# ray-project/kuberay

Measured on NVIDIA H100. Metric: reconciles/sec over 10k RayCluster x 100 pods (batched reconcilePods + status roll-up), higher is better.
Workload: dtype u32

## Files before the change

kuberay_b200/csrc/kr_bucket2.cuh:

```cuda
#pragma once

#include "kr_decide.cuh"

namespace kr {

__device__ __forceinline__ uint32_t inc_epoch_of(const ScratchDev &sc) { return __ldcg(&sc.inc[KR_INC_EPOCH]) + 1u; }

#ifndef KR_D2WARPS
#define KR_D2WARPS 8
#endif
static constexpr int kD2Warps = KR_D2WARPS;
#define KR_ROW_UNHEALTHY (1u << 13)
#define KR_ROW_FRESH (1u << 14)
#define KR_LG_OWNED (1u << 31)

__device__ __forceinline__ uint4 *large_slot(const ScratchDev &sc, uint32_t c, uint32_t rank) {
  if (!sc.lg) return nullptr;
  const uint4 l = __ldcg(&sc.lg[c]);
  const uint32_t j = rank - sc.bucket_stride;
  return j < l.y ? sc.region + l.x + j : nullptr;
}
__device__ __forceinline__ uint4 *rec_slot(const ScratchDev &sc, uint32_t c, uint32_t rank) {
  return rank < sc.bucket_stride ? sc.bucket + (size_t)c * sc.bucket_stride + rank : large_slot(sc, c, rank);
}
// ... 181 lines not shown
    if ((int64_t)count < (int64_t)H) {
#pragma unroll
      for (int k = 0; k < K; k++) if ((mine >> k) & 1u) act[k] = KR_ACT_DELETE_MH_INCOMPLETE;
      gr.flags |= KR_GR_ABORTED; err_arg = (int32_t)count;
      return KR_ERR_MH_INCOMPLETE;
    }
    if (name == KR_ID_EMPTY_STRING) r_empty = n_rep;
    n_rep++;
  }
  for (uint32_t r = lane; r < n_rep; r += 32) s_rep[r] = 0;
  __syncwarp();
#pragma unroll
  for (int k = 0; k < K; k++) {
    if ((((labelled | noname) >> k) & 1u) && (pw[k] & KR_ROW_UNHEALTHY)) {
      const uint32_t r = ((noname >> k) & 1u) ? r_empty : rep[k];
      if (r != KR_MH_NONE) atomicOr(&s_rep[r], KR_MHF_DELETED);
    }
  }
  __syncwarp();
  int32_t n_unh = 0;
#pragma unroll
  for (int k = 0; k < K; k++) {
    const bool hit = ((labelled >> k) & 1u) && (s_rep[rep[k]] & KR_MHF_DELETED);
    if (hit) act[k] = KR_ACT_DELETE_MH_UNHEALTHY;
    n_unh += __popc(__ballot_sync(0xFFFFFFFFu, hit));
  }
  gr.n_unhealthy = n_unh;
  if (wtd_cnt > 0) {
#pragma unroll
    for (int k = 0; k < K; k++) {
      if ((((labelled | noname) >> k) & 1u) && (pw[k] & KR_ROW_WTD_OWN)) {
        const uint32_t r = ((noname >> k) & 1u) ? r_empty : rep[k];
        if (r != KR_MH_NONE) atomicOr(&s_rep[r], KR_MHF_WTD);
      }
    }
    __syncwarp();
    int32_t n_del = 0;
#pragma unroll
    for (int k = 0; k < K; k++) {
      const bool hit = ((labelled >> k) & 1u) && (s_rep[rep[k]] & KR_MHF_WTD);
      if (hit && act[k] == KR_ACT_KEEP) act[k] = KR_ACT_DELETE_MH_WTD;
      n_del += __popc(__ballot_sync(0xFFFFFFFFu, hit));
    }
    gr.flags |= KR_GR_WTD_EXECUTED;
    if (n_del > 0) { gr.flags |= KR_GR_ABORTED; err_arg = n_del; return KR_ERR_MH_WTD; }
  }
  int32_t running = 0;
  for (uint32_t r = lane; r < n_rep; r += 32) running += (s_rep[r] & KR_MHF_DELETED) ? 0 : 1;
  running = __reduce_add_sync(0xFFFFFFFFu, running);
#pragma unroll
  for (int k = 0; k < K; k++) if (((heads >> k) & 1u) && !(s_rep[rep[k]] & KR_MHF_DELETED)) mh_head |= 1u << k;
  gr.n_running = running;
  if (expected % H != 0) { gr.flags |= KR_GR_ABORTED; err_arg = expected; return KR_ERR_MH_NOT_MULTIPLE; }
  const int32_t to_create = expected / H - running;
  gr.diff = to_create;
  if (to_create > 0) gr.n_create = (uint32_t)to_create;
  else if (to_create < 0) {
    if (delete_allowed) {
      const int32_t remove = -to_create;
      int32_t seen = 0;
      for (uint32_t b = 0; b < n_rep && seen < remove; b += 32) {
        const uint32_t r = b + lane;
        const bool ok = r < n_rep && !(s_rep[r] & KR_MHF_DELETED);
        const uint32_t bal = __ballot_sync(0xFFFFFFFFu, ok);
        if (ok && seen + (int32_t)__popc(bal & lt) < remove) s_rep[r] |= KR_MHF_SCALE;
        seen += __popc(bal);
      }
      __syncwarp();
#pragma unroll
      for (int k = 0; k < K; k++) if (((labelled >> k) & 1u) && (s_rep[rep[k]] & KR_MHF_SCALE)) act[k] = KR_ACT_DELETE_MH_SCALE_DOWN;
    } else gr.flags |= KR_GR_RANDOM_DELETE_OFF;
  }
  return KR_ERR_NONE;
}

template <int K, bool kInc = false, bool kMH = false>
__global__ void __launch_bounds__(kD2Warps * 32, (K <= 4 && !kMH ? 32 : 16) / kD2Warps) k_decide2(Decide2Args a) {
  const int phase = kInc ? 2 : a.phase;
  KR_TL(phase ? 12 : 3);
  __shared__ int32_t s_acc[kD2Warps][3][KR_SMEM_GROUPS];
  __shared__ int32_t s_mode[kD2Warps][kMH ? 4 : 3][KR_SMEM_GROUPS];
  __shared__ uint32_t s_list[kD2Warps][32 * K];
  __shared__ uint32_t s_bits[kD2Warps][32];
  const SnapDev &s = a.s;
  const uint32_t warp = threadIdx.x >> 5, lane = threadIdx.x & 31;
  const uint32_t lt = lanemask_lt();
  const uint32_t S = a.sc.bucket_stride;
  uint32_t c = blockIdx.x * kD2Warps + warp;
  bool mine = phase == 0 && c < a.n.n_clusters;
  RecordCI ci{mine ? __ldg(&a.sc.cl_in[32 * (size_t)c + lane]) : 0u};
  pdl_wait(); pdl_trigger();
  if (phase == 1) {
    mine = c < a.r.totals[4];
    if (mine) { c = a.sc.deferred_list[c]; ci.word = __ldg(&a.sc.cl_in[32 * (size_t)c + lane]); }
  } else if (kInc) {
    mine = c < __ldcg(&a.sc.inc[KR_INC_DIRTY]) && !__ldcg(&a.sc.inc[KR_INC_VOID]) && !__ldcg(&a.sc.inc[KR_INC_STRUCTURAL]);
    if (mine) {
      c = a.sc.dirty_list[c];
      ci.word = __ldcg(&a.sc.cl_in[32 * (size_t)c + lane]);
    }
  }
  if (KR_ATTEMPT_VOID(a.r.totals)) mine = false;
  if (ci.group_cnt() > KR_SMEM_GROUPS) mine = false;
  if (kInc && !mine) return;
  uint4 *bucket = a.sc.bucket + (size_t)(mine ? c : 0) * S;
  uint4 dyn = make_uint4(0, 0, 0, 0);
  uint4 recs[K] = {};
  if (mine) {
    dyn = __ldcg(&a.sc.cl_dyn[c]);
#pragma unroll
    for (int k = 0; k < K; k++) if ((uint32_t)(k * 32) + lane < S) recs[k] = __ldcg(&bucket[k * 32 + lane]);
  }
  uint32_t P = dyn.x;
  if (P > S) { mine = false; P = 0; }
  if (kInc) {
    const uint32_t epoch = inc_epoch_of(a.sc);
    const bool lost = dyn.y == epoch;
    uint32_t kept = 0, head_min = 0xFFFFFFFFu;
#pragma unroll
    for (int k = 0; k < K; k++) {
      const uint32_t j = k * 32 + lane;
      bool keep = mine && j < P;
      const bool fresh = keep && (recs[k].y & KR_ROW_FRESH);
      if (keep && lost && !fresh) keep = __ldcg(&a.sc.stamp[recs[k].x]) != epoch;
      const uint32_t bal = __ballot_sync(0xFFFFFFFFu, keep);
      if (keep) {
        uint4 rec = recs[k];
        rec.y &= ~KR_ROW_FRESH;
        const uint32_t to = kept + __popc(bal & lt);
        if (fresh || to != j) { bucket[to] = rec; if (to != j) a.sc.pos[rec.x] = to; }
        if (pp_node_type(rec.y & 0xFFFFu) == KR_NT_HEAD) head_min = min(head_min, rec.x);
      }
      kept += __popc(bal);
    }
    head_min = __reduce_min_sync(0xFFFFFFFFu, head_min);
    __syncwarp();
    unsigned long long raw = 0;
    if (mine) {
      if (lane == 0 && head_min != 0xFFFFFFFFu) raw = ~(((unsigned long long)head_min << 32) | (uint32_t)(aux_lookup(a.sc, head_min) + 1));
      raw = __shfl_sync(0xFFFFFFFFu, raw, 0);
      P = kept;
      dyn = make_uint4(kept, 0u, (uint32_t)raw, (uint32_t)(raw >> 32));
      if (lane == 0) a.sc.cl_dyn[c] = dyn;
#pragma unroll
      for (int k = 0; k < K; k++) if ((uint32_t)(k * 32) + lane < kept) recs[k] = __ldcg(&bucket[k * 32 + lane]);
    }
  }
  const uint32_t cf = ci.flags(), G = ci.group_cnt(), g0 = ci.group_off();
  const uint8_t suspend_status = ci.suspend_status(), ext_err = ci.ext_err_kind(), old_prov = ci.cond_status(KR_COND_PROVISIONED);
  const bool gate = a.f.gate_status_conditions != 0;
  uint32_t old_create = 0;
  if (kInc && mine) {
    for (uint32_t gi = lane; gi < G; gi += 32) old_create += a.r.groups[g0 + gi].n_create;
    old_create = __reduce_add_sync(0xFFFFFFFFu, old_create);
  }
  uint32_t head_pod = 0xFFFFFFFFu;
  int32_t head_aux = -1;
  {
    const unsigned long long raw = ((unsigned long long)dyn.w << 32) | dyn.z;
    if (mine && raw != 0) { const unsigned long long key = ~raw; head_pod = (uint32_t)(key >> 32); head_aux = (int32_t)(uint32_t)key - 1; }
  }
  uint8_t h_ver = KR_VER_EMPTY, h_ast = KR_ANNOT_EMPTY;
  if (head_aux >= 0 && (cf & KR_CF_UPGRADE_RECREATE)) { h_ver = s.h_version_state[head_aux]; h_ast = s.h_annot_state[head_aux]; }
  uint32_t pidx[K], pw[K], ridx[K], act[K];
  uint32_t head_pos = 0xFFFFFFFFu, head_name = 0, head_flags = 0;
#pragma unroll
  for (int k = 0; k < K; k++) {
    const uint32_t i = k * 32 + lane;
    const bool valid = i < P;
    pidx[k] = valid ? recs[k].x : 0xFFFFFFFFu; pw[k] = valid ? recs[k].y : (KR_ROW_NO_GROUP << 16); ridx[k] = valid ? recs[k].z : 0u; act[k] = KR_ACT_KEEP;
    const uint32_t hit = __ballot_sync(0xFFFFFFFFu, valid && recs[k].x == head_pod);
    if (hit) {
      const int src = __ffs(hit) - 1;
      head_pos = k * 32 + src;
      head_name = __shfl_sync(0xFFFFFFFFu, recs[k].w, src); head_flags = __shfl_sync(0xFFFFFFFFu, recs[k].y, src) & 0xFFFFu;
    }
  }
  (void)head_pos;
  int32_t *acc_list = s_acc[warp][0], *acc_unh = s_acc[warp][1], *acc_wtd = s_acc[warp][2];
  int32_t *g_mode = s_mode[warp][0], *g_prefix = s_mode[warp][1], *g_ncreate = s_mode[warp][2], *g_mh_running = s_mode[warp][kMH ? 3 : 2];
  uint32_t mh_head = 0;
  if (lane < KR_SMEM_GROUPS) { acc_list[lane] = 0; acc_unh[lane] = 0; acc_wtd[lane] = 0; g_mode[lane] = GM_UNPROCESSED; g_prefix[lane] = 0; g_ncreate[lane] = 0; }
  __syncwarp();

  int32_t ready = 0, available = 0, n_heads = 0, n0_list = 0, n0_unh = 0, n0_wtd = 0;
  bool all_running = P > 0;
  const uint32_t nchunks = (P + 31) / 32;
#pragma unroll
  for (int k = 0; k < K; k++) {
    if ((uint32_t)k >= nchunks) break;
    const bool valid = (uint32_t)(k * 32) + lane < P;
    const uint32_t w = pw[k], fl = w & 0xFFFFu, slot = valid ? (w >> 16) : KR_ROW_NO_GROUP;
    const uint32_t nt = pp_node_type(fl), ph = pp_phase(fl), rd = pp_ready(fl);
    const bool w_run = valid && nt == KR_NT_WORKER && ph == KR_PHASE_RUNNING;
    available += __popc(__ballot_sync(0xFFFFFFFFu, w_run));
    ready += __popc(__ballot_sync(0xFFFFFFFFu, w_run && rd == KR_COND_TRUE));
    const bool not_ok = valid && (ph != KR_PHASE_RUNNING || rd == KR_COND_FALSE || rd == KR_COND_UNKNOWN);
    if (__any_sync(0xFFFFFFFFu, not_ok)) all_running = false;
    n_heads += __popc(__ballot_sync(0xFFFFFFFFu, valid && nt == KR_NT_HEAD));
    if (G == 1) {
      const bool in0 = slot == 0;
      n0_list += __popc(__ballot_sync(0xFFFFFFFFu, in0));
      n0_unh += __popc(__ballot_sync(0xFFFFFFFFu, in0 && (fl & KR_ROW_UNHEALTHY)));
      n0_wtd += __popc(__ballot_sync(0xFFFFFFFFu, in0 && (fl & KR_ROW_WTD_OWN)));
      continue;
    }
    const uint32_t gkey = (slot < G) ? slot : KR_ROW_NO_GROUP;
    const uint32_t peers = __match_any_sync(0xFFFFFFFFu, gkey);
    if (gkey != KR_ROW_NO_GROUP) {
      const uint32_t ub = __ballot_sync(peers, (fl & KR_ROW_UNHEALTHY) != 0);
      const uint32_t wb = __ballot_sync(peers, (fl & KR_ROW_WTD_OWN) != 0);
      if ((peers & lt) == 0) {
        acc_list[gkey] += __popc(peers);
        acc_unh[gkey] += __popc(ub & peers);
        acc_wtd[gkey] += __popc(wb & peers);
      }
    }
    __syncwarp();
  }
  if (G == 1) { if (lane == 0) { acc_list[0] = n0_list; acc_unh[0] = n0_unh; acc_wtd[0] = n0_wtd; } __syncwarp(); }

  kr_cluster_result cr;
  {
    uint32_t *z = reinterpret_cast<uint32_t *>(&cr);
#pragma unroll
    for (int k = 0; k < (int)(sizeof(cr) / 4); k++) z[k] = 0;
  }
  cr.head_pod_idx = -1; cr.stop_after_group = -1;
  uint8_t all_action = KR_ACT_KEEP;
  bool head_delete = false, run_groups = false, deferred = false, any_prefix = false;
  uint32_t n_create_cluster = 0;
  if (mine) {
    if (cf & KR_CF_SKIP) {
      cr.path = KR_PATH_SKIPPED;
    } else if (ext_err != KR_EXT_ERR_NONE) {
      cr.path = KR_PATH_SKIPPED;
      cr.err_kind = ext_err == KR_EXT_ERR_STATUS_ONLY_NIL ? KR_ERR_NONE : KR_ERR_EXTERNAL;
    } else if (suspend_status == KR_SUSPEND_SUSPENDING || (!gate && (cf & KR_CF_SUSPEND))) {
      cr.path = KR_PATH_SUSPENDING_DELETE_ALL; all_action = KR_ACT_DELETE_ALL_SUSPEND;
    } else if (gate && (suspend_status == KR_SUSPEND_SUSPENDED || (cf & KR_CF_SUSPEND))) {
      cr.path = KR_PATH_SUSPENDED_NOOP;
    } else {
      bool recreate = false;
      if ((cf & KR_CF_UPGRADE_RECREATE) && n_heads > 0) {
        const int32_t aux = head_aux;
        const uint8_t ver = h_ver, ast = h_ast;
        if (ver == KR_VER_DIFFERENT) cr.head_update_annotations = 1;
        else if (ast == KR_ANNOT_OTHER) recreate = true;
        else if (ast == KR_ANNOT_HASH32 && !a.f.skip_hash) {
          if (phase == 0 && !a.spin_hash) {
            deferred = true;
            if (lane == 0) a.sc.deferred_list[atomicAdd(&a.r.totals[4], 1u)] = c;
          } else {
            const uint8_t *ah = s.h_annot_hash + 32 * (size_t)aux;
            const uint32_t *hw = reinterpret_cast<const uint32_t *>(a.r.hash + 32 * (size_t)c);
            if (phase == 0) {
              if (lane == 0) {
                const volatile uint32_t *w7 = hw + 7;
                uint32_t it = 0;
                while (*w7 == 0u && it < 40000u) { __nanosleep(100); it++; }
                if (*w7 == 0u) atomicOr(&a.r.totals[3], KR_TOTALS_HASH_WAIT);
              }
              __syncwarp();
              __threadfence();
            }
            const uint32_t word = __ldcg(&hw[lane >> 2]);
            recreate = __any_sync(0xFFFFFFFFu, ah[lane] != (uint8_t)(word >> (8 * (lane & 3))));
          }
        }
      }
      if (recreate) {
        cr.path = KR_PATH_RECREATE_DELETE_ALL; all_action = KR_ACT_DELETE_ALL_RECREATE;
      } else {
        cr.path = KR_PATH_NORMAL;
        if (!(cf & KR_CF_HEAD_EXPECT_OK)) { cr.head_action = KR_HEAD_EXPECT_PENDING; run_groups = true; }
        else if (n_heads == 1) {
          if (head_flags & KR_ROW_UNHEALTHY) { cr.head_action = KR_HEAD_DELETE; cr.err_kind = KR_ERR_HEAD_DELETED; head_delete = true; }
          else run_groups = true;
        } else if (n_heads == 0) {
          if (old_prov == KR_COND_TRUE && (cf & KR_CF_SKIP_HEAD_RESTART)) cr.head_action = KR_HEAD_SKIP_RESTART;
          else { cr.head_action = KR_HEAD_CREATE; run_groups = true; }
        } else {
          cr.head_action = KR_HEAD_MULTIPLE; cr.err_kind = KR_ERR_MULTIPLE_HEADS; cr.err_arg = n_heads;
        }
      }
    }
    if (run_groups) {
      const bool autoscaling = (cf & KR_CF_AUTOSCALING) != 0;
      cr.stop_after_group = (int32_t)G;
      for (uint32_t gi = 0; gi < G; gi++) {
        const uint32_t g = g0 + gi;
        const bool rec0 = gi == 0;
        const uint32_t gf = rec0 ? ci.g0_flags() : LDG(s.g_flags[g]);
        const int32_t hosts = rec0 ? ci.g0_hosts() : LDG(s.g_num_hosts[g]), g_rep = rec0 ? ci.g0_rep() : LDG(s.g_replicas[g]);
        const int32_t g_mn = rec0 ? ci.g0_min() : LDG(s.g_min[g]), g_mx = rec0 ? ci.g0_max() : LDG(s.g_max[g]);
        kr_group_result gr;
        gr.expected = 0; gr.n_list = 0; gr.n_unhealthy = 0; gr.n_running = 0; gr.diff = 0; gr.n_create = 0; gr.create_off = 0;
        gr.flags = KR_GR_PROCESSED;
        int32_t mode = GM_SKIP, prefix = 0;
        bool abort_here = false;
        if (!(gf & KR_GF_EXPECT_OK)) {
          gr.flags |= KR_GR_EXPECT_PENDING;
        } else {
          const int32_t expected = desired_replicas(g_rep, g_mn, g_mx, hosts, gf);
          const int32_t n_list = acc_list[gi], n_unh = acc_unh[gi], n_wtd = acc_wtd[gi];
          gr.expected = expected; gr.n_list = n_list;
          if (gf & KR_GF_SUSPEND) { gr.flags |= KR_GR_SUSPENDED; mode = GM_SUSPENDED; }
          else if (kMH && hosts > 1 && a.f.gate_multihost_indexing) {
            gr.flags |= KR_GR_MULTIHOST; mode = GM_MULTIHOST;
            int32_t earg = 0;
            const int ek = decide_multihost2<K>(s, gi, expected, hosts, !autoscaling || a.f.env_random_pod_delete, LDG(s.g_wtd_cnt[g]), pidx, pw, act, mh_head,
                                                s_list[warp], gr, earg, lane);
            if (ek != KR_ERR_NONE) { cr.err_kind = (uint8_t)ek; cr.err_arg = earg; abort_here = true; }
            if (lane == 0) g_mh_running[gi] = gr.n_running;
          }
          else if (n_unh > 0) {
            gr.n_unhealthy = n_unh; gr.flags |= KR_GR_ABORTED; mode = GM_UNHEALTHY;
            cr.err_kind = KR_ERR_UNHEALTHY_WORKERS; cr.err_arg = n_unh; abort_here = true;
          } else {
            gr.flags |= KR_GR_WTD_EXECUTED; mode = GM_NORMAL;
            const int32_t running = n_list - n_wtd;
            const int32_t diff = expected - running;
            gr.n_running = running; gr.diff = diff;
            if (diff > 0) gr.n_create = (uint32_t)diff;
            else if (diff < 0) {
              if (!autoscaling || a.f.env_random_pod_delete) {
                const long long remove = -(long long)diff;
                if (remove > running) {
                  prefix = running; gr.flags |= KR_GR_ABORTED;
                  cr.err_kind = KR_ERR_NEGATIVE_EXPECTED; cr.err_arg = expected; abort_here = true;
                } else prefix = (int32_t)remove;
              } else gr.flags |= KR_GR_RANDOM_DELETE_OFF;
            }
          }
        }
        any_prefix |= prefix > 0;
        n_create_cluster += gr.n_create;
        __syncwarp();
        if (lane == 0) {
          g_mode[gi] = mode; g_prefix[gi] = prefix; g_ncreate[gi] = (int32_t)gr.n_create;
          a.r.groups[g] = gr;
        }
        if (abort_here) { cr.stop_after_group = (int32_t)gi; break; }
      }
    }
    {
      const int32_t reached = ((cf & KR_CF_SKIP) || !run_groups) ? 0 : (cr.stop_after_group == (int32_t)G ? (int32_t)G : cr.stop_after_group + 1);
      for (uint32_t gi = reached + lane; gi < G; gi += 32) {
        kr_group_result z; z.expected = 0; z.n_list = 0; z.n_unhealthy = 0; z.n_running = 0; z.diff = 0; z.n_create = 0; z.create_off = 0; z.flags = 0;
        a.r.groups[g0 + gi] = z;
      }
    }
  }
  __syncwarp();

  uint32_t cand = 0;
  if (mine) {
#pragma unroll
    for (int k = 0; k < K; k++) {
      if ((uint32_t)k >= nchunks) break;
      const bool valid = (uint32_t)(k * 32) + lane < P;
      const uint32_t w = pw[k], fl = w & 0xFFFFu;
      const uint32_t gkey = (valid && run_groups && (w >> 16) < G) ? (w >> 16) : KR_ROW_NO_GROUP;
      const int32_t mode = (gkey != KR_ROW_NO_GROUP) ? g_mode[gkey] : GM_UNPROCESSED;
      uint32_t ac = KR_ACT_KEEP;
      if (all_action != KR_ACT_KEEP) ac = valid ? all_action : (uint32_t)KR_ACT_KEEP;
      else if (head_delete) { if (valid && pidx[k] == head_pod) ac = KR_ACT_DELETE_HEAD; }
      else if (mode == GM_SUSPENDED) ac = KR_ACT_DELETE_GROUP_SUSPEND;
      else if (kMH && mode == GM_MULTIHOST) ac = act[k];
      else if (mode == GM_UNHEALTHY) { if (fl & KR_ROW_UNHEALTHY) ac = KR_ACT_DELETE_UNHEALTHY; }
      else if (mode == GM_NORMAL) {
        if (fl & KR_ROW_WTD_OWN) ac = KR_ACT_DELETE_WTD;
        else cand |= 1u << k;
      }
      act[k] = ac;
    }
    if (any_prefix) {
      for (uint32_t gi = 0; gi < G; gi++) {
        const int32_t pre = g_prefix[gi];
        if (pre <= 0) continue;
        if (pre <= 8) {
          for (int32_t it = 0; it < pre; it++) {
            uint32_t m = 0xFFFFFFFFu;
#pragma unroll
            for (int k = 0; k < K; k++)
              if (((cand >> k) & 1u) && (pw[k] >> 16) == gi && act[k] == KR_ACT_KEEP) m = min(m, pidx[k]);
            const uint32_t wm = __reduce_min_sync(0xFFFFFFFFu, m);
            if (wm == 0xFFFFFFFFu) break;
#pragma unroll
            for (int k = 0; k < K; k++)
              if (((cand >> k) & 1u) && pidx[k] == wm) act[k] = KR_ACT_DELETE_RANDOM;
          }
        } else {
          uint32_t nc = 0;
#pragma unroll
          for (int k = 0; k < K; k++) {
            const bool isc = ((cand >> k) & 1u) && (pw[k] >> 16) == gi;
            const uint32_t bal = __ballot_sync(0xFFFFFFFFu, isc);
            if (isc) s_list[warp][nc + __popc(bal & lt)] = pidx[k];
            nc += __popc(bal);
          }
          __syncwarp();
#pragma unroll
          for (int k = 0; k < K; k++) {
            const bool isc = ((cand >> k) & 1u) && (pw[k] >> 16) == gi;
            if (!__any_sync(0xFFFFFFFFu, isc)) continue;
            uint32_t rank = 0;
            for (uint32_t i = 0; i < nc; i++) rank += s_list[warp][i] < pidx[k] ? 1u : 0u;
            if (isc && (int32_t)rank < pre) act[k] = KR_ACT_DELETE_RANDOM;
          }
          __syncwarp();
        }
      }
    }
  }
  uint32_t n_act = 0;
  uint32_t arank[K];
#pragma unroll
  for (int k = 0; k < K; k++) {
    arank[k] = 0;
    const bool isa = act[k] != KR_ACT_KEEP;
    const uint32_t bal = __ballot_sync(0xFFFFFFFFu, isa);
    if (isa) s_list[warp][n_act + __popc(bal & lt)] = pidx[k];
    n_act += __popc(bal);
  }
  __syncwarp();
  if (n_act > 1) {
#pragma unroll
    for (int k = 0; k < K; k++) {
      const bool isa = act[k] != KR_ACT_KEEP;
      if (!__any_sync(0xFFFFFFFFu, isa)) continue;
      uint32_t rank = 0;
      for (uint32_t i = 0; i < n_act; i++) rank += s_list[warp][i] < pidx[k] ? 1u : 0u;
      arank[k] = rank;
    }
  }

  if (!(cf & KR_CF_SKIP))
    status_rollup(a.s, a.f, ci, cr, P, (uint32_t)n_heads, n_heads > 0 ? (int32_t)head_pod : -1, head_aux, head_name, ready, available, all_running);
  if (mine && lane == 0) a.r.clusters[c] = cr;

  const uint32_t slots = deferred ? P : n_act;
  uint32_t act_off = 0, create_off = 0;
  if (phase == 0) {
    unsigned long long base = 0;
    if (mine && lane == 0) {
      if (slots | n_create_cluster) base = atomicAdd(reinterpret_cast<unsigned long long *>(&a.r.totals[8]), ((unsigned long long)n_create_cluster << 32) | slots);
      if (n_act) atomicAdd(&a.r.totals[2], n_act);
      if (n_create_cluster) atomicAdd(&a.r.totals[6], n_create_cluster);
    }
    base = __shfl_sync(0xFFFFFFFFu, base, 0);
    act_off = (uint32_t)base; create_off = (uint32_t)(base >> 32);
    if (mine && lane == 0) {
      a.r.act_start[c] = act_off; a.r.act_cnt[c] = n_act;
      if (deferred) a.sc.cact[c] = n_create_cluster;
      a.sc.act_res[c] = slots; a.sc.cre_res[c] = n_create_cluster;
    }
  } else if (kInc) {
    unsigned long long base = 0;
    uint32_t need = 0;
    if (mine && lane == 0) {
      const uint32_t old_act = a.r.act_cnt[c];
      need = (n_act > a.sc.act_res[c] ? 1u : 0u) | (n_create_cluster > a.sc.cre_res[c] ? 2u : 0u);
      if (need) base = atomicAdd(reinterpret_cast<unsigned long long *>(&a.r.totals[8]), ((unsigned long long)((need & 2u) ? n_create_cluster : 0u) << 32) | ((need & 1u) ? n_act : 0u));
      if ((need & 1u) && (uint64_t)(uint32_t)base + n_act > a.n.n_pods) a.sc.inc[KR_INC_VOID] = 1u;
      if ((need & 2u) && (uint64_t)(uint32_t)(base >> 32) + n_create_cluster > a.create_cap) a.sc.inc[KR_INC_VOID] = 1u;
      if (n_act != old_act) atomicAdd(&a.r.totals[2], n_act - old_act);
      if (n_create_cluster != old_create) atomicAdd(&a.r.totals[6], n_create_cluster - old_create);
    }
    base = __shfl_sync(0xFFFFFFFFu, base, 0); need = __shfl_sync(0xFFFFFFFFu, need, 0);
    if (mine) {
      act_off = (need & 1u) ? (uint32_t)base : a.r.act_start[c];
      create_off = (need & 2u) ? (uint32_t)(base >> 32) : (G ? a.sc.gcreate[g0] : 0u);
      if ((need & 1u) && (uint64_t)act_off + n_act > a.n.n_pods) mine = false;
      if ((need & 2u) && (uint64_t)create_off + n_create_cluster > a.create_cap) mine = false;
      if (mine && lane == 0) {
        a.r.act_start[c] = act_off; a.r.act_cnt[c] = n_act;
        if (need & 1u) a.sc.act_res[c] = n_act;
        if (need & 2u) a.sc.cre_res[c] = n_create_cluster;
      }
    }
  } else if (mine) {
    act_off = a.r.act_start[c];
    if (lane == 0) {
      const uint32_t old_act = a.r.act_cnt[c], old_create = a.sc.cact[c];
      a.r.act_cnt[c] = n_act;
      if (n_act != old_act) atomicAdd(&a.r.totals[2], n_act - old_act);
      if (n_create_cluster != old_create) atomicAdd(&a.r.totals[6], n_create_cluster - old_create);
    }
  }
  if (!mine) return;
#pragma unroll
  for (int k = 0; k < K; k++)
    if (act[k] != KR_ACT_KEEP) { a.r.act_pod_idx[act_off + arank[k]] = pidx[k]; a.r.act_code[act_off + arank[k]] = (uint8_t)act[k]; }
  if (phase == 1 || n_create_cluster) {
    uint32_t off = create_off;
    for (uint32_t gi = 0; gi < G; gi++) {
      const uint32_t g = g0 + gi;
      const uint32_t want = (uint32_t)g_ncreate[gi];
      if (phase == 1) {
        off = a.sc.gcreate[g];
      }
      if (lane == 0) { a.r.groups[g].create_off = off; if (phase != 1) a.sc.gcreate[g] = off; }
      if (want == 0) continue;
      if ((uint64_t)off + want > a.create_cap) { off += want; continue; }
      int32_t *out = a.r.create_idx + off;
      if (!a.f.gate_multihost_indexing) {
        for (uint32_t k2 = lane; k2 < want; k2 += 32) out[k2] = -1;
      } else {
        const bool mh = kMH && g_mode[gi] == GM_MULTIHOST;
        const uint64_t bound = (uint64_t)(mh ? g_mh_running[gi] : acc_list[gi] - acc_wtd[gi]) + want;
        uint32_t written = 0;
        for (uint64_t w0 = 0; w0 < bound && written < want; w0 += 1024) {
          s_bits[warp][lane] = 0;
          __syncwarp();
#pragma unroll
          for (int k = 0; k < K; k++) {
            if ((pw[k] >> 16) == gi && (pw[k] & KR_PP_HAS_REPLICA_IDX) && (mh ? ((mh_head >> k) & 1u) != 0 : (act[k] == KR_ACT_KEEP && pidx[k] != 0xFFFFFFFFu))) {
              const int32_t idx = (int32_t)ridx[k];
              if (idx >= 0 && (uint64_t)idx >= w0 && (uint64_t)idx < w0 + 1024 && (uint64_t)idx < bound)
                atomicOr(&s_bits[warp][(idx - w0) >> 5], 1u << ((idx - w0) & 31));
            }
          }
          __syncwarp();
          const uint32_t word = s_bits[warp][lane];
          const uint64_t wbase = w0 + 32ull * lane;
          uint32_t freeb = ~word;
          if (wbase >= bound) freeb = 0;
          else if (bound - wbase < 32) freeb &= (1u << (uint32_t)(bound - wbase)) - 1;
          const uint32_t cnt = __popc(freeb);
          uint32_t x = cnt;
#pragma unroll
          for (int d = 1; d < 32; d <<= 1) { const uint32_t y = __shfl_up_sync(0xFFFFFFFFu, x, d); if (lane >= (uint32_t)d) x += y; }
          uint32_t pos = written + x - cnt;
          while (freeb && pos < want) {
            const uint32_t bit = __ffs(freeb) - 1;
            freeb &= freeb - 1;
            out[pos++] = (int32_t)(wbase + bit);
          }
          written += __shfl_sync(0xFFFFFFFFu, x, 31);
          __syncwarp();
        }
      }
      off += want;
    }
  } else if (G) {
    for (uint32_t gi = lane; gi < G; gi += 32) { a.r.groups[g0 + gi].create_off = create_off; a.sc.gcreate[g0 + gi] = create_off; }
  }
  if (kInc) {
    __syncwarp();
    stage_cluster(a, blockIdx.x * kD2Warps + warp, c, act_off, n_act, g0, G, lane);
  }
}

}
```

kuberay_b200/csrc/kr_decide.cuh:

```cuda
#pragma once

#include "kr_bucket.cuh"

namespace kr {


#define KR_SMEM_GROUPS 32
static constexpr int kDecideWarps = 4;

enum { GM_UNPROCESSED = 0, GM_SKIP = 1, GM_SUSPENDED = 2, GM_UNHEALTHY = 3, GM_NORMAL = 4, GM_MULTIHOST = 5 };

__device__ __forceinline__ uint32_t warp_lower_bound(const uint32_t *__restrict__ a, uint32_t n, uint32_t v, uint32_t lane) {
  uint32_t lo = 0, hi = n;
  while (hi - lo > 32) {
    uint32_t step = (hi - lo + 31) / 32;
    uint32_t idx = lo + (lane + 1) * step - 1;
    bool ge = (idx >= hi) ? true : (__ldg(&a[idx]) >= v);
    uint32_t b = __ballot_sync(0xFFFFFFFFu, ge);
    if (b == 0) return hi;
    uint32_t first = __ffs(b) - 1;
    uint32_t nlo = lo + first * step, nhi = min(hi, lo + (first + 1) * step - 1);
    lo = nlo; hi = nhi;
  }
  uint32_t idx = lo + lane;
  bool ge = (idx >= hi) ? true : (__ldg(&a[idx]) >= v);
  uint32_t b = __ballot_sync(0xFFFFFFFFu, ge);
  return b ? lo + (__ffs(b) - 1) : hi;
}

struct DecideArgs {
  SnapDev s; ScratchDev sc; ResDev r; Sizes n; kr_flags f;
  const uint32_t *sorted_keys;
  const uint32_t *unsorted;
  int fast;
  int phase;
};

struct ColumnsCI {
  const SnapDev &s; uint32_t c;
  __device__ __forceinline__ uint32_t flags() const { return s.c_flags[c]; }
  __device__ __forceinline__ uint8_t ext_err_kind() const { return s.c_ext_err_kind[c]; }
  __device__ __forceinline__ uint32_t ext_err_msg() const { return s.c_ext_err_msg_id[c]; }
  __device__ __forceinline__ uint8_t cond_status(int k) const { return s.c_old_cond_status[5 * (size_t)c + k]; }
  __device__ __forceinline__ uint8_t cond_variant(int k) const { return s.c_old_cond_variant[5 * (size_t)c + k]; }
  __device__ __forceinline__ uint32_t reason() const { return s.c_old_cond_reason_id[c]; }
  __device__ __forceinline__ uint32_t msg(int k) const { return s.c_old_cond_msg_id[2 * (size_t)c + k]; }
  __device__ __forceinline__ uint32_t group_cnt() const { return s.c_group_cnt[c]; }
  __device__ __forceinline__ uint32_t group_off() const { return s.c_group_off[c]; }
  __device__ __forceinline__ uint8_t svc_count() const { return s.c_svc_count[c]; }
  __device__ __forceinline__ uint8_t svc_ip_kind() const { return s.c_svc_ip_kind[c]; }
  __device__ __forceinline__ uint32_t svc_ip() const { return s.c_svc_ip_id[c]; }
  __device__ __forceinline__ uint32_t svc_name() const { return s.c_svc_name_id[c]; }
  __device__ __forceinline__ uint8_t old_state() const { return s.c_old_state[c]; }
  __device__ __forceinline__ uint8_t suspend_status() const { return s.c_suspend_status[c]; }
  __device__ __forceinline__ int32_t old_count(int k) const { return s.c_old_counts[5 * (size_t)c + k]; }
  __device__ __forceinline__ uint32_t old_head(int k) const { return s.c_old_head_ids[4 * (size_t)c + k]; }
  __device__ __forceinline__ bool has_group0() const { return false; }
  __device__ __forceinline__ uint32_t g0_flags() const { return 0; }
  __device__ __forceinline__ int32_t g0_rep() const { return 0; }
  __device__ __forceinline__ int32_t g0_min() const { return 0; }
  __device__ __forceinline__ int32_t g0_max() const { return 0; }
  __device__ __forceinline__ int32_t g0_hosts() const { return 0; }
};
struct RecordCI {
  uint32_t word;
  __device__ __forceinline__ uint32_t w(int i) const { return __shfl_sync(0xFFFFFFFFu, word, i); }
  __device__ __forceinline__ uint8_t byte(int i, int b) const { return (uint8_t)(w(i) >> (8 * b)); }
  __device__ __forceinline__ uint32_t flags() const { return w(KR_CI_FLAGS); }
  __device__ __forceinline__ uint8_t ext_err_kind() const { return byte(KR_CI_B0, 1); }
  __device__ __forceinline__ uint32_t ext_err_msg() const { return w(KR_CI_EXT_MSG); }
  __device__ __forceinline__ uint8_t cond_status(int k) const { return k < 3 ? byte(KR_CI_B1, 1 + k) : byte(KR_CI_B2, k - 3); }
  __device__ __forceinline__ uint8_t cond_variant(int k) const { return k < 2 ? byte(KR_CI_B2, 2 + k) : byte(KR_CI_B3, k - 2); }
  __device__ __forceinline__ uint32_t reason() const { return w(KR_CI_REASON); }
  __device__ __forceinline__ uint32_t msg(int k) const { return w(KR_CI_MSG + k); }
  __device__ __forceinline__ uint32_t group_cnt() const { return w(KR_CI_GCNT); }
  __device__ __forceinline__ uint32_t group_off() const { return w(KR_CI_GOFF); }
  __device__ __forceinline__ uint8_t svc_count() const { return byte(KR_CI_B0, 3); }
  __device__ __forceinline__ uint8_t svc_ip_kind() const { return byte(KR_CI_B1, 0); }
  __device__ __forceinline__ uint32_t svc_ip() const { return w(KR_CI_SVC_IP); }
  __device__ __forceinline__ uint32_t svc_name() const { return w(KR_CI_SVC_NAME); }
  __device__ __forceinline__ uint8_t old_state() const { return byte(KR_CI_B0, 2); }
  __device__ __forceinline__ uint8_t suspend_status() const { return byte(KR_CI_B0, 0); }
  __device__ __forceinline__ int32_t old_count(int k) const { return (int32_t)w(KR_CI_CNT + k); }
  __device__ __forceinline__ uint32_t old_head(int k) const { return w(KR_CI_HEAD + k); }
  __device__ __forceinline__ bool has_group0() const { return true; }
  __device__ __forceinline__ uint32_t g0_flags() const { return w(KR_CI_G0_FLAGS); }
  __device__ __forceinline__ int32_t g0_rep() const { return (int32_t)w(KR_CI_G0_REP); }
  __device__ __forceinline__ int32_t g0_min() const { return (int32_t)w(KR_CI_G0_MIN); }
  __device__ __forceinline__ int32_t g0_max() const { return (int32_t)w(KR_CI_G0_MAX); }
  __device__ __forceinline__ int32_t g0_hosts() const { return (int32_t)w(KR_CI_G0_HOSTS); }
};

template <class CI>
__device__ __forceinline__ void status_rollup(const SnapDev &s, const kr_flags &f, const CI &ci, kr_cluster_result &cr, uint32_t P, uint32_t n_heads,
                                              int32_t head_pod, int32_t aux, uint32_t head_name_id, int32_t ready, int32_t available, bool all_running) {
  const uint32_t cf = ci.flags();
  const bool gate = f.gate_status_conditions != 0;
  const bool reconcile_err = cr.err_kind != KR_ERR_NONE;
  const uint8_t ek = ci.ext_err_kind();
  uint8_t cst[KR_NUM_CONDS], cvr[KR_NUM_CONDS], ocst[KR_NUM_CONDS], ocvr[KR_NUM_CONDS];
#pragma unroll
  for (int k = 0; k < KR_NUM_CONDS; k++) { ocst[k] = cst[k] = ci.cond_status(k); ocvr[k] = cvr[k] = ci.cond_variant(k); }
  const uint32_t old_reason = ci.reason(), old_msg0 = ci.msg(0), old_msg1 = ci.msg(1);
  uint32_t hpr_reason = old_reason, hpr_msg = old_msg0, rf_msg = old_msg1;
  if (gate) {
    if (reconcile_err) {
      if (ek >= KR_EXT_ERR_FAILED_DELETE_ALL_PODS && ek <= KR_EXT_ERR_FAILED_CREATE_WORKER_POD) {
        cst[KR_COND_REPLICA_FAILURE] = KR_COND_TRUE; cvr[KR_COND_REPLICA_FAILURE] = ek; rf_msg = ci.ext_err_msg();
      }
    } else {
      cst[KR_COND_REPLICA_FAILURE] = KR_COND_ABSENT; cvr[KR_COND_REPLICA_FAILURE] = KR_CV_NONE; rf_msg = 0;
    }
  }
  int32_t desired = 0, minr = 0; long long maxr = 0;
  const uint32_t G = ci.group_cnt(), g0 = ci.group_off();
  for (uint32_t gi = 0; gi < G; gi++) {
    const uint32_t g = g0 + gi;
    const bool rec = gi == 0 && ci.has_group0();
    const uint32_t gf = rec ? ci.g0_flags() : s.g_flags[g];
    const int32_t hosts = rec ? ci.g0_hosts() : s.g_num_hosts[g], g_rep = rec ? ci.g0_rep() : s.g_replicas[g];
    const int32_t g_mn = rec ? ci.g0_min() : s.g_min[g], g_mx = rec ? ci.g0_max() : s.g_max[g];
    desired = (int32_t)((uint32_t)desired + (uint32_t)desired_replicas(g_rep, g_mn, g_mx, hosts, gf));
    if (gf & KR_GF_SUSPEND) continue;
    int32_t mn = (gf & KR_GF_MIN_NIL) ? 0 : g_mn;
    int32_t mx = (gf & KR_GF_MAX_NIL) ? INT32_MAX : g_mx;
    minr = (int32_t)((uint32_t)minr + (uint32_t)mn * (uint32_t)hosts);
    maxr += (long long)mx * (long long)hosts;
  }
  int32_t maxc = maxr > INT32_MAX ? INT32_MAX : (maxr < INT32_MIN ? INT32_MIN : (int32_t)maxr);

  cr.n_pods = (int32_t)P; cr.n_heads = (int32_t)n_heads; cr.head_pod_idx = head_pod;
  uint8_t serr = KR_SERR_NONE;
  const uint8_t svc_count = ci.svc_count(), svc_ip_kind = ci.svc_ip_kind();
  if (n_heads > 1) serr = KR_SERR_MULTIPLE_HEADS;
  else if (svc_count == 0) serr = KR_SERR_NO_HEAD_SERVICE;
  else if (svc_count > 1) serr = KR_SERR_MULTIPLE_HEAD_SERVICES;
  else if (svc_ip_kind == KR_SVCIP_EMPTY) serr = KR_SERR_EMPTY_SERVICE_IP;
  cr.status_err = serr;
  if (serr != KR_SERR_NONE) return;

  const uint8_t old_state = ci.old_state();
  uint8_t new_state = old_state;
  bool reason_cleared = false;
  if (!reconcile_err && (long long)P == (long long)desired + 1 && all_running) { new_state = KR_STATE_READY; reason_cleared = true; }

  uint32_t head_pod_ip = 0, head_pod_name = 0;
  if (n_heads != 1) aux = -1;
  if (n_heads == 1) {
    head_pod_ip = aux >= 0 ? s.h_pod_ip_id[aux] : 0;
    head_pod_name = head_name_id;
  }
  if (gate) {
    if (n_heads == 0) {
      cst[KR_COND_HEAD_POD_READY] = KR_COND_FALSE; cvr[KR_COND_HEAD_POD_READY] = KR_CV_HEAD_NOT_FOUND;
      hpr_reason = f.id_head_not_found_reason; hpr_msg = f.id_head_not_found_msg;
    } else {
      cst[KR_COND_HEAD_POD_READY] = aux >= 0 ? s.h_ready_status[aux] : (uint8_t)KR_COND_FALSE;
      cvr[KR_COND_HEAD_POD_READY] = KR_CV_HEAD_FROM_POD;
      hpr_reason = aux >= 0 ? s.h_ready_reason_id[aux] : 0; hpr_msg = aux >= 0 ? s.h_ready_msg_id[aux] : 0;
    }
    const uint8_t ss = ci.suspend_status();
    if (cst[KR_COND_PROVISIONED] != KR_COND_TRUE && ss != KR_SUSPEND_SUSPENDED) {
      if (all_running) { cst[KR_COND_PROVISIONED] = KR_COND_TRUE; cvr[KR_COND_PROVISIONED] = KR_CV_PROV_ALL_READY; }
      else { cst[KR_COND_PROVISIONED] = KR_COND_FALSE; cvr[KR_COND_PROVISIONED] = KR_CV_PROV_PROVISIONING; }
    }
    if (ss == KR_SUSPEND_SUSPENDING) {
      if (P == 0) {
        cst[KR_COND_PROVISIONED] = KR_COND_FALSE; cvr[KR_COND_PROVISIONED] = KR_CV_PROV_SUSPENDED;
        cst[KR_COND_SUSPENDING] = KR_COND_FALSE; cvr[KR_COND_SUSPENDING] = KR_CV_CANONICAL;
        cst[KR_COND_SUSPENDED] = KR_COND_TRUE; cvr[KR_COND_SUSPENDED] = KR_CV_CANONICAL;
      }
    } else if (ss == KR_SUSPEND_SUSPENDED) {
      if (cf & KR_CF_SUSPEND_SET_FALSE) { cst[KR_COND_SUSPENDED] = KR_COND_FALSE; cvr[KR_COND_SUSPENDED] = KR_CV_CANONICAL; }
    } else {
      cst[KR_COND_SUSPENDED] = KR_COND_FALSE; cvr[KR_COND_SUSPENDED] = KR_CV_CANONICAL;
      cst[KR_COND_SUSPENDING] = (cf & KR_CF_SUSPEND) ? KR_COND_TRUE : KR_COND_FALSE; cvr[KR_COND_SUSPENDING] = KR_CV_CANONICAL;
    }
  }
  if ((cf & KR_CF_SUSPEND) && P == 0) new_state = KR_STATE_SUSPENDED;

  uint32_t svc_ip = ci.svc_ip();
  if (svc_ip_kind == KR_SVCIP_NONE) svc_ip = (n_heads == 1) ? head_pod_ip : 0;
  uint32_t head_ids[4] = {head_pod_ip, svc_ip, head_pod_name, ci.svc_name()};

  cr.new_state = new_state;
  cr.state_changed = new_state != old_state;
  cr.status_flags = (reason_cleared ? KR_SF_READY_BRANCH : 0u) | (all_running ? KR_SF_ALL_PODS_RUNNING : 0u);
  cr.counts[0] = ready; cr.counts[1] = available; cr.counts[2] = desired; cr.counts[3] = minr; cr.counts[4] = maxc;
#pragma unroll
  for (int k = 0; k < KR_NUM_CONDS; k++) { cr.cond_status[k] = cst[k]; cr.cond_variant[k] = cvr[k]; }
  cr.head_ready_reason_id = hpr_reason; cr.head_ready_msg_id = hpr_msg;
#pragma unroll
  for (int k = 0; k < 4; k++) cr.head_ids[k] = head_ids[k];

  bool inc = new_state != old_state;
  if (reason_cleared && (cf & KR_CF_OLD_REASON_NONEMPTY)) inc = true;
#pragma unroll
  for (int k = 0; k < 5; k++) if (ci.old_count(k) != cr.counts[k]) inc = true;
  if (cf & KR_CF_ENDPOINTS_CHANGED) inc = true;
#pragma unroll
  for (int k = 0; k < 4; k++) if (ci.old_head(k) != head_ids[k]) inc = true;
#pragma unroll
  for (int k = 0; k < KR_NUM_CONDS; k++) {
    if (ocst[k] != cst[k]) { inc = true; continue; }
    if (cst[k] == KR_COND_ABSENT) continue;
    if (k == KR_COND_HEAD_POD_READY) {
      if (old_reason != hpr_reason || old_msg0 != hpr_msg) inc = true;
    } else if (k == KR_COND_REPLICA_FAILURE) {
      if (ocvr[k] != cvr[k] || old_msg1 != rf_msg) inc = true;
    } else if (ocvr[k] != cvr[k]) inc = true;
  }
  cr.needs_status_write = inc ? 1 : 0;
}

#define KR_MH_NONE 0xFFFFFFFFu
#define KR_MH_UNASSIGNED 0xFFFFFFFEu
#define KR_MH_NOREP 0xFFFFFFFDu
#define KR_MHF_DELETED 1u
#define KR_MHF_WTD 2u
#define KR_MHF_SCALE 4u
__device__ int decide_multihost(const DecideArgs &a, uint32_t slot, uint32_t seg0, uint32_t seg1, int32_t expected, int32_t H,
                                bool delete_allowed, uint32_t wtd_cnt, kr_group_result &gr, int32_t &err_arg, uint32_t lane) {
  uint32_t *rep = a.sc.mh_rep, *name = a.sc.mh_name, *meta = a.sc.mh_meta, *cnt = a.sc.mh_cnt, *flg = a.sc.mh_flg;
  uint8_t *act = a.sc.mh_act, *headv = a.sc.mh_head;
  const uint32_t lt = lanemask_lt();
  for (uint32_t b = seg0; b < seg1; b += 32) {
    uint32_t i = b + lane;
    if (i < seg1) {
      uint4 row = a.sc.rows[a.r.sorted_pod_idx[i]];
      bool member = (row.w >> 16) == slot;
      rep[i] = member ? (row.y ? KR_MH_UNASSIGNED : KR_MH_NOREP) : KR_MH_NONE;
      if (member) { name[i] = row.y; meta[i] = row.w & 0xFFFFu; act[i] = KR_ACT_KEEP; headv[i] = 0; }
    }
  }
  __syncwarp();
  uint32_t cursor = seg0, first_incomplete = KR_MH_NONE, m_empty = KR_MH_NONE;
  int32_t incomplete_cnt = 0;
  while (true) {
    uint32_t m = KR_MH_NONE;
    for (uint32_t b = cursor; b < seg1; b += 32) {
      uint32_t i = b + lane;
      uint32_t bal = __ballot_sync(0xFFFFFFFFu, i < seg1 && rep[i] == KR_MH_UNASSIGNED);
      if (bal) { m = b + (__ffs(bal) - 1); break; }
    }
    if (m == KR_MH_NONE) break;
    const uint32_t nm = name[m];
    uint32_t count = 0;
    for (uint32_t b = m; b < seg1; b += 32) {
      uint32_t i = b + lane;
      bool hit = i < seg1 && rep[i] == KR_MH_UNASSIGNED && name[i] == nm;
      if (hit) rep[i] = m;
      count += __popc(__ballot_sync(0xFFFFFFFFu, hit));
    }
    if (lane == 0) { cnt[m] = count; flg[m] = 0; }
    if (nm == KR_ID_EMPTY_STRING) m_empty = m;
    if ((int64_t)count < (int64_t)H && first_incomplete == KR_MH_NONE) { first_incomplete = m; incomplete_cnt = (int32_t)count; }
    cursor = m + 1;
    __syncwarp();
  }
  if (first_incomplete != KR_MH_NONE) {
    for (uint32_t b = seg0; b < seg1; b += 32) { uint32_t i = b + lane; if (i < seg1 && rep[i] == first_incomplete) act[i] = KR_ACT_DELETE_MH_INCOMPLETE; }
    gr.flags |= KR_GR_ABORTED; err_arg = incomplete_cnt;
    __syncwarp();
    return KR_ERR_MH_INCOMPLETE;
  }
  for (uint32_t b = seg0; b < seg1; b += 32) {
    uint32_t i = b + lane;
    if (i < seg1 && rep[i] != KR_MH_NONE && should_delete(meta[i])) {
      uint32_t r = rep[i] == KR_MH_NOREP ? m_empty : rep[i];
      if (r != KR_MH_NONE) atomicOr(&flg[r], KR_MHF_DELETED);
    }
  }
  __syncwarp();
  int32_t n_unh = 0;
  for (uint32_t b = seg0; b < seg1; b += 32) {
    uint32_t i = b + lane;
    bool hit = i < seg1 && rep[i] < KR_MH_NOREP && (flg[rep[i]] & KR_MHF_DELETED);
    if (hit) act[i] = KR_ACT_DELETE_MH_UNHEALTHY;
    n_unh += __popc(__ballot_sync(0xFFFFFFFFu, hit));
  }
  gr.n_unhealthy = n_unh;
  if (wtd_cnt > 0) {
    for (uint32_t b = seg0; b < seg1; b += 32) {
      uint32_t i = b + lane;
      if (i < seg1 && rep[i] != KR_MH_NONE && (meta[i] & KR_ROW_WTD_OWN)) {
        uint32_t r = rep[i] == KR_MH_NOREP ? m_empty : rep[i];
        if (r != KR_MH_NONE) atomicOr(&flg[r], KR_MHF_WTD);
      }
    }
    __syncwarp();
    int32_t n_del = 0;
    for (uint32_t b = seg0; b < seg1; b += 32) {
      uint32_t i = b + lane;
// ... 406 lines not shown
```

Measured before the change: 80.53 million.

## Move per-warp cluster record and result into shared memory to cut registers

Stages the per-cluster input record in shared memory so field reads become shared loads instead of warp shuffles. The cluster result is built in a shared volatile struct and written out cooperatively, one word per lane, instead of by lane 0. Two values that were held across the whole kernel, the replica index and the head name, are now reloaded from global memory where they are used, and the status roll-up compares against the stored record rather than keeping copies. The aim is to lower register pressure and raise occupancy, at the cost of more shared memory per block, extra global reloads and volatile shared accesses.

Result: faster. 83.97 million (median of 6 runs) (+4.3%).

```diff
diff --git a/kuberay_b200/csrc/kr_bucket2.cuh b/kuberay_b200/csrc/kr_bucket2.cuh
--- a/kuberay_b200/csrc/kr_bucket2.cuh
+++ b/kuberay_b200/csrc/kr_bucket2.cuh
@@ -287,24 +287,31 @@
   __shared__ int32_t s_mode[kD2Warps][kMH ? 4 : 3][KR_SMEM_GROUPS];
   __shared__ uint32_t s_list[kD2Warps][32 * K];
   __shared__ uint32_t s_bits[kD2Warps][32];
+  __shared__ uint32_t s_in[kD2Warps][32];
+  __shared__ kr_cluster_result s_cr[kD2Warps];
+  __shared__ uint32_t s_deferred[kD2Warps];
+  __shared__ uint32_t s_old_create[kInc ? kD2Warps : 1];
   const SnapDev &s = a.s;
   const uint32_t warp = threadIdx.x >> 5, lane = threadIdx.x & 31;
   const uint32_t lt = lanemask_lt();
   const uint32_t S = a.sc.bucket_stride;
   uint32_t c = blockIdx.x * kD2Warps + warp;
   bool mine = phase == 0 && c < a.n.n_clusters;
-  RecordCI ci{mine ? __ldg(&a.sc.cl_in[32 * (size_t)c + lane]) : 0u};
+  uint32_t in_word = mine ? __ldg(&a.sc.cl_in[32 * (size_t)c + lane]) : 0u;
   pdl_wait(); pdl_trigger();
   if (phase == 1) {
     mine = c < a.r.totals[4];
-    if (mine) { c = a.sc.deferred_list[c]; ci.word = __ldg(&a.sc.cl_in[32 * (size_t)c + lane]); }
+    if (mine) { c = a.sc.deferred_list[c]; in_word = __ldg(&a.sc.cl_in[32 * (size_t)c + lane]); }
   } else if (kInc) {
     mine = c < __ldcg(&a.sc.inc[KR_INC_DIRTY]) && !__ldcg(&a.sc.inc[KR_INC_VOID]) && !__ldcg(&a.sc.inc[KR_INC_STRUCTURAL]);
     if (mine) {
       c = a.sc.dirty_list[c];
-      ci.word = __ldcg(&a.sc.cl_in[32 * (size_t)c + lane]);
-    }
-  }
+      in_word = __ldcg(&a.sc.cl_in[32 * (size_t)c + lane]);
+    }
+  }
+  s_in[warp][lane] = in_word;
+  __syncwarp();
+  const RecordCI ci{s_in[warp]};
   if (KR_ATTEMPT_VOID(a.r.totals)) mine = false;
   if (ci.group_cnt() > KR_SMEM_GROUPS) mine = false;
   if (kInc && !mine) return;
@@ -347,17 +354,17 @@
       P = kept;
       dyn = make_uint4(kept, 0u, (uint32_t)raw, (uint32_t)(raw >> 32));
       if (lane == 0) a.sc.cl_dyn[c] = dyn;
-#pragma unroll
-      for (int k = 0; k < K; k++) if ((uint32_t)(k * 32) + lane < kept) recs[k] = __ldcg(&bucket[k * 32 + lane]);
-    }
+    }
+#pragma unroll
+    for (int k = 0; k < K; k++) recs[k] = mine && (uint32_t)(k * 32) + lane < kept ? __ldcg(&bucket[k * 32 + lane]) : make_uint4(0, 0, 0, 0);
   }
   const uint32_t cf = ci.flags(), G = ci.group_cnt(), g0 = ci.group_off();
   const uint8_t suspend_status = ci.suspend_status(), ext_err = ci.ext_err_kind(), old_prov = ci.cond_status(KR_COND_PROVISIONED);
   const bool gate = a.f.gate_status_conditions != 0;
-  uint32_t old_create = 0;
   if (kInc && mine) {
+    uint32_t old_create = 0;
     for (uint32_t gi = lane; gi < G; gi += 32) old_create += a.r.groups[g0 + gi].n_create;
-    old_create = __reduce_add_sync(0xFFFFFFFFu, old_create);
+    s_old_create[warp] = __reduce_add_sync(0xFFFFFFFFu, old_create);
   }
   uint32_t head_pod = 0xFFFFFFFFu;
   int32_t head_aux = -1;
@@ -367,21 +374,20 @@
   }
   uint8_t h_ver = KR_VER_EMPTY, h_ast = KR_ANNOT_EMPTY;
   if (head_aux >= 0 && (cf & KR_CF_UPGRADE_RECREATE)) { h_ver = s.h_version_state[head_aux]; h_ast = s.h_annot_state[head_aux]; }
-  uint32_t pidx[K], pw[K], ridx[K], act[K];
-  uint32_t head_pos = 0xFFFFFFFFu, head_name = 0, head_flags = 0;
+  uint32_t pidx[K], pw[K], act[K];
+  uint32_t head_pos = 0xFFFFFFFFu, head_flags = 0;
 #pragma unroll
   for (int k = 0; k < K; k++) {
     const uint32_t i = k * 32 + lane;
     const bool valid = i < P;
-    pidx[k] = valid ? recs[k].x : 0xFFFFFFFFu; pw[k] = valid ? recs[k].y : (KR_ROW_NO_GROUP << 16); ridx[k] = valid ? recs[k].z : 0u; act[k] = KR_ACT_KEEP;
+    pidx[k] = valid ? recs[k].x : 0xFFFFFFFFu; pw[k] = valid ? recs[k].y : (KR_ROW_NO_GROUP << 16); act[k] = KR_ACT_KEEP;
     const uint32_t hit = __ballot_sync(0xFFFFFFFFu, valid && recs[k].x == head_pod);
     if (hit) {
       const int src = __ffs(hit) - 1;
       head_pos = k * 32 + src;
-      head_name = __shfl_sync(0xFFFFFFFFu, recs[k].w, src); head_flags = __shfl_sync(0xFFFFFFFFu, recs[k].y, src) & 0xFFFFu;
-    }
-  }
-  (void)head_pos;
+      head_flags = __shfl_sync(0xFFFFFFFFu, recs[k].y, src) & 0xFFFFu;
+    }
+  }
   int32_t *acc_list = s_acc[warp][0], *acc_unh = s_acc[warp][1], *acc_wtd = s_acc[warp][2];
   int32_t *g_mode = s_mode[warp][0], *g_prefix = s_mode[warp][1], *g_ncreate = s_mode[warp][2], *g_mh_running = s_mode[warp][kMH ? 3 : 2];
   uint32_t mh_head = 0;
@@ -425,15 +431,16 @@
   }
   if (G == 1) { if (lane == 0) { acc_list[0] = n0_list; acc_unh[0] = n0_unh; acc_wtd[0] = n0_wtd; } __syncwarp(); }
 
-  kr_cluster_result cr;
-  {
-    uint32_t *z = reinterpret_cast<uint32_t *>(&cr);
-#pragma unroll
-    for (int k = 0; k < (int)(sizeof(cr) / 4); k++) z[k] = 0;
-  }
-  cr.head_pod_idx = -1; cr.stop_after_group = -1;
+  volatile kr_cluster_result &cr = s_cr[warp];
+  static_assert(sizeof(kr_cluster_result) % 4 == 0 && sizeof(kr_cluster_result) / 4 <= 32, "one word of the result record per lane");
+  if (lane < sizeof(kr_cluster_result) / 4) {
+    const bool neg = lane == offsetof(kr_cluster_result, head_pod_idx) / 4 || lane == offsetof(kr_cluster_result, stop_after_group) / 4;
+    reinterpret_cast<volatile uint32_t *>(&cr)[lane] = neg ? 0xFFFFFFFFu : 0u;
+  }
+  if (lane == 0) s_deferred[warp] = 0;
+  __syncwarp();
   uint8_t all_action = KR_ACT_KEEP;
-  bool head_delete = false, run_groups = false, deferred = false, any_prefix = false;
+  bool head_delete = false, run_groups = false, any_prefix = false;
   uint32_t n_create_cluster = 0;
   if (mine) {
     if (cf & KR_CF_SKIP) {
@@ -454,7 +461,7 @@
         else if (ast == KR_ANNOT_OTHER) recreate = true;
         else if (ast == KR_ANNOT_HASH32 && !a.f.skip_hash) {
           if (phase == 0 && !a.spin_hash) {
-            deferred = true;
+            s_deferred[warp] = 1;
             if (lane == 0) a.sc.deferred_list[atomicAdd(&a.r.totals[4], 1u)] = c;
           } else {
             const uint8_t *ah = s.h_annot_hash + 32 * (size_t)aux;
@@ -619,6 +626,14 @@
       }
     }
   }
+  if (!(cf & KR_CF_SKIP)) {
+    const uint32_t head_name = (n_heads == 1 && head_pos != 0xFFFFFFFFu) ? __ldcg(&a.sc.bucket[(size_t)c * S + head_pos].w) : 0u;
+    status_rollup(a.s, a.f, ci, cr, P, (uint32_t)n_heads, n_heads > 0 ? (int32_t)head_pod : -1, head_aux, head_name, ready, available, all_running);
+  }
+  __syncwarp();
+  if (mine && lane < sizeof(kr_cluster_result) / 4)
+    reinterpret_cast<uint32_t *>(&a.r.clusters[c])[lane] = reinterpret_cast<const volatile uint32_t *>(&cr)[lane];
+
   uint32_t n_act = 0;
   uint32_t arank[K];
 #pragma unroll
@@ -641,10 +656,7 @@
     }
   }
 
-  if (!(cf & KR_CF_SKIP))
-    status_rollup(a.s, a.f, ci, cr, P, (uint32_t)n_heads, n_heads > 0 ? (int32_t)head_pod : -1, head_aux, head_name, ready, available, all_running);
-  if (mine && lane == 0) a.r.clusters[c] = cr;
-
+  const bool deferred = s_deferred[warp] != 0;
   const uint32_t slots = deferred ? P : n_act;
   uint32_t act_off = 0, create_off = 0;
   if (phase == 0) {
@@ -665,7 +677,7 @@
     unsigned long long base = 0;
     uint32_t need = 0;
     if (mine && lane == 0) {
-      const uint32_t old_act = a.r.act_cnt[c];
+      const uint32_t old_act = a.r.act_cnt[c], old_create = s_old_create[warp];
       need = (n_act > a.sc.act_res[c] ? 1u : 0u) | (n_create_cluster > a.sc.cre_res[c] ? 2u : 0u);
       if (need) base = atomicAdd(reinterpret_cast<unsigned long long *>(&a.r.totals[8]), ((unsigned long long)((need & 2u) ? n_create_cluster : 0u) << 32) | ((need & 1u) ? n_act : 0u));
       if ((need & 1u) && (uint64_t)(uint32_t)base + n_act > a.n.n_pods) a.sc.inc[KR_INC_VOID] = 1u;
@@ -722,7 +734,7 @@
 #pragma unroll
           for (int k = 0; k < K; k++) {
             if ((pw[k] >> 16) == gi && (pw[k] & KR_PP_HAS_REPLICA_IDX) && (mh ? ((mh_head >> k) & 1u) != 0 : (act[k] == KR_ACT_KEEP && pidx[k] != 0xFFFFFFFFu))) {
-              const int32_t idx = (int32_t)ridx[k];
+              const int32_t idx = (int32_t)__ldcg(&a.sc.bucket[(size_t)c * S + k * 32 + lane].z);
               if (idx >= 0 && (uint64_t)idx >= w0 && (uint64_t)idx < w0 + 1024 && (uint64_t)idx < bound)
                 atomicOr(&s_bits[warp][(idx - w0) >> 5], 1u << ((idx - w0) & 31));
             }
diff --git a/kuberay_b200/csrc/kr_decide.cuh b/kuberay_b200/csrc/kr_decide.cuh
--- a/kuberay_b200/csrc/kr_decide.cuh
+++ b/kuberay_b200/csrc/kr_decide.cuh
@@ -63,8 +63,8 @@
   __device__ __forceinline__ int32_t g0_hosts() const { return 0; }
 };
 struct RecordCI {
-  uint32_t word;
-  __device__ __forceinline__ uint32_t w(int i) const { return __shfl_sync(0xFFFFFFFFu, word, i); }
+  const uint32_t *rec;
+  __device__ __forceinline__ uint32_t w(int i) const { return rec[i]; }
   __device__ __forceinline__ uint8_t byte(int i, int b) const { return (uint8_t)(w(i) >> (8 * b)); }
   __device__ __forceinline__ uint32_t flags() const { return w(KR_CI_FLAGS); }
   __device__ __forceinline__ uint8_t ext_err_kind() const { return byte(KR_CI_B0, 1); }
@@ -91,18 +91,17 @@
   __device__ __forceinline__ int32_t g0_hosts() const { return (int32_t)w(KR_CI_G0_HOSTS); }
 };
 
-template <class CI>
-__device__ __forceinline__ void status_rollup(const SnapDev &s, const kr_flags &f, const CI &ci, kr_cluster_result &cr, uint32_t P, uint32_t n_heads,
+template <class CI, class CR>
+__device__ __forceinline__ void status_rollup(const SnapDev &s, const kr_flags &f, const CI &ci, CR &cr, uint32_t P, uint32_t n_heads,
                                               int32_t head_pod, int32_t aux, uint32_t head_name_id, int32_t ready, int32_t available, bool all_running) {
   const uint32_t cf = ci.flags();
   const bool gate = f.gate_status_conditions != 0;
   const bool reconcile_err = cr.err_kind != KR_ERR_NONE;
   const uint8_t ek = ci.ext_err_kind();
-  uint8_t cst[KR_NUM_CONDS], cvr[KR_NUM_CONDS], ocst[KR_NUM_CONDS], ocvr[KR_NUM_CONDS];
-#pragma unroll
-  for (int k = 0; k < KR_NUM_CONDS; k++) { ocst[k] = cst[k] = ci.cond_status(k); ocvr[k] = cvr[k] = ci.cond_variant(k); }
-  const uint32_t old_reason = ci.reason(), old_msg0 = ci.msg(0), old_msg1 = ci.msg(1);
-  uint32_t hpr_reason = old_reason, hpr_msg = old_msg0, rf_msg = old_msg1;
+  uint8_t cst[KR_NUM_CONDS], cvr[KR_NUM_CONDS];
+#pragma unroll
+  for (int k = 0; k < KR_NUM_CONDS; k++) { cst[k] = ci.cond_status(k); cvr[k] = ci.cond_variant(k); }
+  uint32_t hpr_reason = ci.reason(), hpr_msg = ci.msg(0), rf_msg = ci.msg(1);
   if (gate) {
     if (reconcile_err) {
       if (ek >= KR_EXT_ERR_FAILED_DELETE_ALL_PODS && ek <= KR_EXT_ERR_FAILED_CREATE_WORKER_POD) {
@@ -202,13 +201,14 @@
   for (int k = 0; k < 4; k++) if (ci.old_head(k) != head_ids[k]) inc = true;
 #pragma unroll
   for (int k = 0; k < KR_NUM_CONDS; k++) {
-    if (ocst[k] != cst[k]) { inc = true; continue; }
-    if (cst[k] == KR_COND_ABSENT) continue;
+    const uint8_t st = cr.cond_status[k];
+    if (ci.cond_status(k) != st) { inc = true; continue; }
+    if (st == KR_COND_ABSENT) continue;
     if (k == KR_COND_HEAD_POD_READY) {
-      if (old_reason != hpr_reason || old_msg0 != hpr_msg) inc = true;
+      if (ci.reason() != cr.head_ready_reason_id || ci.msg(0) != cr.head_ready_msg_id) inc = true;
     } else if (k == KR_COND_REPLICA_FAILURE) {
-      if (ocvr[k] != cvr[k] || old_msg1 != rf_msg) inc = true;
-    } else if (ocvr[k] != cvr[k]) inc = true;
+      if (ci.cond_variant(k) != cr.cond_variant[k] || ci.msg(1) != rf_msg) inc = true;
+    } else if (ci.cond_variant(k) != cr.cond_variant[k]) inc = true;
   }
   cr.needs_status_write = inc ? 1 : 0;
 }
```
